# kxhit/vMAP

Measured on NVIDIA H100. Metric: training-step rays/sec at n_obj x n_rays x n_samples, higher is better.
Workload: dtype fp16

## Files before the change

### vmap_b200/csrc/k_step_fused.cuh

```cuda
#pragma once
#include <string>
#include <cmath>
#include "common.cuh"
#include "k_step_fp32.cuh"
#include "umma_ptx.cuh"
#include "k_umma_image.cuh"

struct FusedExtra {
  float* partials;
  unsigned int* finish_sync;
  const int* counts_in;
  int* counts_pub;
  int fuse_adam;
  float* p; float* m; float* v;
  __half* image_out; const int* img_index; int img_halves;
  int* step_counter;
  float step_size, bc2_sqrt;
  double lr, b1d, b2d;
  float log_b1, log_b2;
  const float2* bc_table;
  int bc_n;
  float lr_wd, one_m_b1, b2, one_m_b2, eps;
  int guard_loss;
  int* status;
// ... 20 lines not shown
  int on[3];
  int fin, skip;
  float step_size, bc2_sqrt;
  float lsum[4][4];
};
static_assert(sizeof(Misc) <= MISC_BYTES, "Misc");

__device__ __forceinline__ uint32_t pack_relu_h2(float lo, float hi) {
  uint32_t r;
  asm("cvt.rn.relu.satfinite.f16x2.f32 %0, %1, %2;" : "=r"(r) : "f"(hi), "f"(lo));
  return r;
}

__device__ __forceinline__ int wg_base(const VmbLayout& L, int blk, int lane, int& ld) {
  ld = 1;
  switch (blk) {
    case 0: {
      if (lane >= 96) return -1;
      const int j = um::emb1_col_to_j(lane);
      if (j == -2) return L.o_bin;
      if (j < 0) return -1;
      ld = VMB_E1; return L.o_Win + j;
    }
    case 1:
      if (lane < 32) { ld = 32; return L.o_Wm1 + lane; }
      return lane == 64 ? L.o_bm1 : -1;
    case 2: {
      if (lane < 32) { ld = 32 + VMB_E1; return L.o_Wcat + lane; }
      const int j = um::emb1_col_to_j(lane - 32);
      if (j == -2) return L.o_bcat;
      if (j < 0) return -1;
      ld = 32 + VMB_E1; return L.o_Wcat + 32 + j;
    }
    case 3:
      if (lane < 32) { ld = 32; return L.o_Wm2 + lane; }
      return lane == 64 + 42 ? L.o_bm2 : -1;
    default: {
      if (lane < 32) { ld = 32 + L.e2; return L.o_Wcl + lane; }
      if (lane >= 80) return -1;
      const int j2 = um::emb2_col_to_j2(lane - 32);
      if (j2 == -2) return L.o_bcl;
      if (j2 < 0) return -1;
      ld = 32 + L.e2; return L.o_Wcl + 32 + j2;
    }
  }
}

struct Mma {
  uint32_t a16, w16;
  int mh;

  static __device__ __forceinline__ uint64_t mk(uint32_t base16, uint32_t off, uint32_t lbo, uint32_t sbo) {
    const uint32_t lo = ((base16 + (off >> 4)) & 0x3FFFu) | ((lbo >> 4) << 16);
    return ((uint64_t)(sbo >> 4) << 32) | lo;
  }
  __device__ __forceinline__ uint64_t a_k(int fg, int ks) const { return mk(a16, fg * FGB + mh * 1024 + ks * 4096, 2048, 128); }
  __device__ __forceinline__ uint64_t xa_mn(int fg, int ks) const { return mk(a16, (fg + 8 * mh) * FGB + ks * 256, 128, 2048); }
  __device__ __forceinline__ uint64_t xb_mn(int fg, int ks) const { return mk(a16, fg * FGB + ks * 256, 128, 2048); }
  __device__ __forceinline__ uint64_t w_k(int off, int ks) const { return mk(w16, off + ks * 1024, 512, 128); }
  __device__ __forceinline__ uint64_t w16_k(int off, int ks) const { return mk(w16, off + ks * 512, 256, 128); }
  __device__ __forceinline__ uint64_t w_mn(int off, int ks) const { return mk(w16, off + ks * 256, 128, 512); }
  __device__ __forceinline__ uint64_t w16_mn(int off) const { return mk(w16, off, 128, 256); }

  __device__ __forceinline__ void wgrad32(float (&d)[16], int fgX, int fgDY) const {
#pragma unroll
    for (int ks = 0; ks < 8; ++ks) ptx::wgmma_n32<1, 1>(d, xa_mn(fgX, ks), xb_mn(fgDY, ks), 1u);
  }
  __device__ __forceinline__ void wgrad16(float (&d)[8], int fgX, int fgDY) const {
#pragma unroll
    for (int ks = 0; ks < 8; ++ks) ptx::wgmma_n16<1, 1>(d, xa_mn(fgX, ks), xb_mn(fgDY, ks), 1u);
  }
};

constexpr int MAX_CTAS = 192;
struct Ranges { int begin[MAX_CTAS + 1]; };
__device__ __forceinline__ int cta_of_pair(const Ranges& rg, int G, int pair) {
  int lo = 0, hi = G - 1;
  while (lo < hi) { const int mid = (lo + hi + 1) >> 1; if (rg.begin[mid] <= pair) lo = mid; else hi = mid - 1; }
  return lo;
}

}

template <int SC>
__global__ void __launch_bounds__(uf::NT, 1)
k_step_fused(StepParams a, FusedExtra x, VmbLayout L, const unsigned char* image, const __grid_constant__ uf::Ranges rg, int tpo, int npo, int nr, int rpw) {
  using namespace uf;
  extern __shared__ __align__(1024) unsigned char smem[];
  Misc* misc = reinterpret_cast<Misc*>(smem + SM_MISC);
  int* cnt = reinterpret_cast<int*>(smem + SM_CNT);
  const int tid = threadIdx.x, warp = tid >> 5, lane = tid & 31;
  const int S = SC ? SC : a.S, R = a.R;

  if (tid == 0) {
    ptx::mbar_init(&misc->wbar, 1);
    misc->on[0] = misc->on[1] = misc->on[2] = 1;
    ptx::mbar_init_fence();
  }
  const int G = gridDim.x;
  const long long gt_begin = rg.begin[blockIdx.x], gt_end = rg.begin[blockIdx.x + 1];
  __syncthreads();
  if (tid == 0 && gt_begin < gt_end) {
    ptx::mbar_arrive_expect_tx(&misc->wbar, um::IMG_BYTES);
    ptx::bulk_g2s(smem + SM_W, image + (size_t)(gt_begin / npo) * um::IMG_BYTES, um::IMG_BYTES, &misc->wbar);
  }
  const bool pub_counts = !x.counts_in && !a.fwd_only;
  unsigned int* gbar = x.finish_sync;
  if (pub_counts) {
    for (int b = blockIdx.x; b < a.B; b += G) {
      if (tid < 3) cnt[tid] = 0;
      __syncthreads();
      const unsigned char* s = a.sem + (size_t)b * a.sem_stride;
      const unsigned char* m = a.mask + (size_t)b * a.mask_stride;
      const bool vec = (((size_t)s | (size_t)m) & 3) == 0;
      const int nw = vec ? (R >> 2) : 0;
      auto nzb = [](uint32_t v) { v |= v >> 4; v |= v >> 2; v |= v >> 1; return v & 0x01010101u; };
      int nd = 0, no = 0, ns = 0;
      for (int w = tid; w < nw; w += NT) {
        const uint32_t sv = __ldg(reinterpret_cast<const uint32_t*>(s) + w), mv = __ldg(reinterpret_cast<const uint32_t*>(m) + w);
        const uint32_t o = nzb(sv);
        no += __popc(o); nd += __popc(o & nzb(mv)); ns += __popc(nzb(sv ^ 0x02020202u));
      }
      for (int r = (nw << 2) + tid; r < R; r += NT) {
        const int sv = s[r], mo = sv != 0;
        nd += (m[r] != 0) & mo; no += mo; ns += sv != 2;
      }
#pragma unroll
      for (int o = 16; o > 0; o >>= 1) {
        nd += __shfl_xor_sync(0xffffffffu, nd, o); no += __shfl_xor_sync(0xffffffffu, no, o); ns += __shfl_xor_sync(0xffffffffu, ns, o);
      }
      if (lane == 0) { atomicAdd(&cnt[0], nd); atomicAdd(&cnt[1], no); atomicAdd(&cnt[2], ns); }
      __syncthreads();
      if (tid == 0) {
        for (int k = 0; k < 3; ++k) {
          x.counts_pub[b * 4 + k] = cnt[k];
          if (cnt[k] == 0) atomicOr(&gbar[3 + k], 1u);
        }
        __threadfence();
        atomicAdd(&gbar[2], 1u);
      }
      __syncthreads();
    }
  } else if (!a.fwd_only) {
    for (int i = tid; i < a.B * 3; i += NT) {
      const int c = x.counts_in[(i / 3) * 4 + (i % 3)];
      cnt[i] = c;
      if (c == 0) misc->on[i % 3] = 0;
    }
  }
  __syncthreads();

  uint32_t wpar = 0;

  const int p = tid & 127, hsel = tid >> 7;
  const int quad = (warp & 3);
  const int rw = lane / S, sidx = lane - rw * S;
  const bool lane_used = rw < rpw;
  const int ray_in_tile = quad * rpw + rw;
  const int seg_lo = lane - sidx;
  unsigned char* act = smem + SM_ACT0;
  unsigned char* eg = smem + SM_EG;
  float* hd = reinterpret_cast<float*>(smem + SM_HD);
  const float* wf = reinterpret_cast<const float*>(smem + SM_W + um::IMG_F32);
  const float* Bd = wf + um::F_DIRS;
  const int cq = lane & 3, fr0 = 64 * hsel + 16 * quad + (lane >> 2);
  Mma mm;
  mm.a16 = ptx::smem_u32(act) >> 4;
  mm.w16 = ptx::smem_u32(smem + SM_W) >> 4;
  mm.mh = hsel;
  float wIN[16] = {}, wM1[16] = {}, wCAT[16] = {}, wM2[16] = {}, wCL[16] = {}, wHD[8] = {}, wDB[8] = {};
  const float on_d = misc->on[0] ? 1.f : 0.f, on_c = misc->on[1] ? 1.f : 0.f, on_o = misc->on[2] ? 1.f : 0.f;
  float w_d = 0.f, w_c = 0.f, w_o = 0.f;
  bool cnt_ready = !pub_counts;

  auto finish_rows = [&](int b, int i_lo, int i_hi, bool owner) -> int {
    const int c_first = cta_of_pair(rg, G, b * npo), c_last = cta_of_pair(rg, G, (b + 1) * npo - 1);
    const int nseg = c_last - c_first + 1;
    const float* P0 = x.partials + (size_t)(c_first + b) * L.stride;
    const size_t row = (size_t)b * L.stride;
    const int n4 = L.stride >> 2;
    const bool upd = a.backward != 0;
    if (warp == 0) {
      float s = 0.f;
      if (nseg <= 10) {
        const int k = lane / 3, j = lane - 3 * k;
        const float v = (k < nseg) ? __ldcg(P0 + (size_t)k * L.stride + L.P + j) : 0.f;
        for (int kk = 0; kk < nseg; ++kk) s += __shfl_sync(0xffffffffu, v, kk * 3 + (lane < 3 ? lane : 0));
      } else if (lane < 3) {
        for (int k = 0; k < nseg; ++k) s += __ldcg(P0 + (size_t)k * L.stride + L.P + lane);
      }
      const float l_d = __shfl_sync(0xffffffffu, s, 0), l_c = __shfl_sync(0xffffffffu, s, 1), l_o = __shfl_sync(0xffffffffu, s, 2);
      if (lane == 0) {
        const float tot = l_d + a.cs * l_c + a.os * l_o;
        if (owner) { float* lt = a.loss_terms + b * 4; lt[0] = l_d; lt[1] = l_c; lt[2] = l_o; lt[3] = tot; }
        int bad = 0;
        if (x.guard_loss) {
          if (l_d > 100000.f || l_c > 100000.f || l_o > 100000.f) bad |= 1;
          if (!(tot == tot) || fabsf(tot) > 3.0e38f) bad |= 2;
          if (bad && x.status && owner) atomicOr(x.status, bad);
        }
        misc->skip = bad;
        if (x.fuse_adam && x.step_counter) {
          const int t = x.step_counter[b] + 1;
          if (t < x.bc_n) {
            const float2 bc = x.bc_table[t];
            misc->step_size = (float)x.lr / bc.x;
            misc->bc2_sqrt = bc.y;
          } else {
            misc->step_size = (float)x.lr / (-expm1f((float)t * x.log_b1));
            misc->bc2_sqrt = sqrtf(-expm1f((float)t * x.log_b2));
          }
        } else {
          misc->step_size = x.step_size; misc->bc2_sqrt = x.bc2_sqrt;
        }
      }
    }
    __syncthreads();
    const int sk = misc->skip;
    if (upd && !(sk && x.fuse_adam)) {
      const float step_size = misc->step_size, bc2_sqrt = misc->bc2_sqrt;
      for (int c4 = i_lo + tid; c4 < i_hi; c4 += NT) {
        const float4* src = reinterpret_cast<const float4*>(P0) + c4;
        float4 pp, mm = make_float4(0.f, 0.f, 0.f, 0.f), vv = mm;
        if (x.fuse_adam) {
          pp = *(reinterpret_cast<const float4*>(x.p + row) + c4);
          mm = *(reinterpret_cast<const float4*>(x.m + row) + c4);
          vv = *(reinterpret_cast<const float4*>(x.v + row) + c4);
        } else {
          pp = *(reinterpret_cast<const float4*>(a.grads + row) + c4);
        }
        float4 gsum = make_float4(0.f, 0.f, 0.f, 0.f);
#pragma unroll 1
        for (int k0 = 0; k0 < nseg; k0 += 4) {
          float4 u[4];
#pragma unroll
// ... 43 lines not shown
    gt += p1 - p0;
    const int t0 = 2 * p0, t1 = min(2 * p1, tpo);

    um::mbar_wait_or_trap(&misc->wbar, wpar);
    wpar ^= 1;

    float ls_d = 0.f, ls_c = 0.f, ls_o = 0.f;
    {
    const float isc = 1.0f / a.scale[b];
    bool seg_w = false;
    if (x.counts_in && !a.fwd_only) {
      w_d = on_d / ((float)cnt[b * 3 + 0] + 1e-10f);
      w_c = on_c / ((float)cnt[b * 3 + 1] + 1e-10f);
      w_o = on_o / ((float)cnt[b * 3 + 2] + 1e-10f);
    }

#define OPERANDS_READY() do { ptx::fence_async_smem(); __syncthreads(); ptx::wgmma_fence(); } while (0)
#define MMA_DONE() do { ptx::wgmma_commit(); ptx::wgmma_wait<0>(); } while (0)
    auto epi_relu = [&](const float (&v)[16], int bias_off, int fg) {
#pragma unroll
      for (int j = 0; j < 4; ++j) {
        const float2 bb = *reinterpret_cast<const float2*>(wf + bias_off + 8 * j + 2 * cq);
        unsigned char* dst = act + (fg + j) * FGB + fr0 * 16 + cq * 4;
        *reinterpret_cast<uint32_t*>(dst) = pack_relu_h2(v[4 * j] + bb.x, v[4 * j + 1] + bb.y);
        *reinterpret_cast<uint32_t*>(dst + 128) = pack_relu_h2(v[4 * j + 2] + bb.x, v[4 * j + 3] + bb.y);
      }
    };
    auto epi_dgrad = [&](const float (&v)[16], int fg_h, int fg_out) {
#pragma unroll
      for (int j = 0; j < 4; ++j) {
        const int off = j * FGB + fr0 * 16 + cq * 4;
        const uint32_t h0 = *reinterpret_cast<const uint32_t*>(act + fg_h * FGB + off);
        const uint32_t h1 = *reinterpret_cast<const uint32_t*>(act + fg_h * FGB + off + 128);
        *reinterpret_cast<uint32_t*>(act + fg_out * FGB + off) = um::gate_h2(um::pack_h2(v[4 * j], v[4 * j + 1]), h0);
        *reinterpret_cast<uint32_t*>(act + fg_out * FGB + off + 128) = um::gate_h2(um::pack_h2(v[4 * j + 2], v[4 * j + 3]), h1);
      }
    };
    auto eg_store = [&](const auto& v, int blk0) {
      constexpr int NJ = (int)(sizeof(v) / 16);
#pragma unroll
      for (int j = 0; j < NJ; ++j) {
        float* d = reinterpret_cast<float*>(eg + (blk0 + 2 * j + (cq >> 1)) * FGB + fr0 * 16 + (cq & 1) * 8);
        *reinterpret_cast<float2*>(d) = make_float2(v[4 * j], v[4 * j + 1]);
        *reinterpret_cast<float2*>(d + 32) = make_float2(v[4 * j + 2], v[4 * j + 3]);
      }
    };
    auto eg_load8 = [&](int blk, float (&o)[8]) {
      const float4 u0 = *reinterpret_cast<const float4*>(eg + blk * FGB + p * 16);
      const float4 u1 = *reinterpret_cast<const float4*>(eg + (blk + 1) * FGB + p * 16);
      o[0] = u0.x; o[1] = u0.y; o[2] = u0.z; o[3] = u0.w; o[4] = u1.x; o[5] = u1.y; o[6] = u1.z; o[7] = u1.w;
    };

    float nx = 0.f, ny = 0.f, nz = 0.f, nzv = 0.f, n_gd = 0.f, n_c0 = 0.f, n_c1 = 0.f, n_c2 = 0.f;
    int n_sem = 0, n_msk = 0;
    bool n_live = false;
    const float* pcs_b = a.pcs + (size_t)b * a.pcs_stride + (size_t)sidx * 3;
    const float* z_b = a.z + (size_t)b * a.z_stride + sidx;
    const float* gd_b = a.gt_depth + (size_t)b * a.gt_depth_stride;
    const float* gc_b = a.gt_colour + (size_t)b * a.gt_colour_stride;
    const unsigned char* sem_b = a.sem + (size_t)b * a.sem_stride;
    const unsigned char* msk_b = a.mask + (size_t)b * a.mask_stride;
    const bool want_targets = hsel == 0 && !a.fwd_only;
    auto prefetch = [&](int t) {
      nx = ny = nz = nzv = 0.f; n_gd = n_c0 = n_c1 = n_c2 = 0.f; n_sem = 0; n_msk = 0; n_live = false;
      if (t >= t1 || !lane_used) return;
      const int ray = t * nr + ray_in_tile;
      if (ray >= R) return;
      const size_t pi = (size_t)ray * S;
      const float* pp = pcs_b + pi * 3;
      nx = pp[0]; ny = pp[1]; nz = pp[2];
      if (want_targets) {
        nzv = z_b[pi];
        n_gd = gd_b[ray];
        const float* gcp = gc_b + (size_t)ray * 3;
        n_c0 = gcp[0]; n_c1 = gcp[1]; n_c2 = gcp[2];
        n_sem = sem_b[ray];
        n_msk = msk_b[ray];
      }
      n_live = true;
    };
    prefetch(t0);

    for (int t = t0; t < t1; ++t) {
      const int ray = t * nr + ray_in_tile;
      const float t0x = nx * isc, t1x = ny * isc, t2x = nz * isc, zv = nzv;
      const uint64_t tp0 = um::pk2(t0x, t0x), tp1 = um::pk2(t1x, t1x), tp2 = um::pk2(t2x, t2x);
      const float gd = n_gd, gc0 = n_c0, gc1 = n_c1, gc2 = n_c2;
      const int sv = n_sem, mv = n_msk;
      const bool live = n_live;
      prefetch(t + 1);
      {
        uint4* e1 = reinterpret_cast<uint4*>(act + FG_E1 * FGB + p * 16);
        uint4* e2 = reinterpret_cast<uint4*>(act + FG_E2 * FGB + p * 16);
        const int q0 = hsel ? 3 : 0, q1 = hsel ? 5 : 3;
        uint64_t s01, s23, c01, c23;
        {
          uint64_t pj01, pj23;
          um::project4(Bd, q0, tp0, tp1, tp2, pj01, pj23);
          um::sincos4_x2(pj01, pj23, s01, s23, c01, c23);
        }
#pragma unroll 1
        for (int q = q0; q < q1; ++q) {
          float sv[4][6];
          uint64_t ns01 = 0, ns23 = 0, nc01 = 0, nc23 = 0;
          if (q + 1 < q1) {
            uint64_t pj01, pj23;
            um::project4(Bd, q + 1, tp0, tp1, tp2, pj01, pj23);
            um::sincos4_x2(pj01, pj23, ns01, ns23, nc01, nc23);
          }
          um::sin_doubling4_x2(s01, s23, c01, c23, sv);
          s01 = ns01; s23 = ns23; c01 = nc01; c23 = nc23;
          const uint4 ua = make_uint4(um::pack_h2(sv[0][0], sv[0][1]), um::pack_h2(sv[0][2], sv[0][3]), um::pack_h2(sv[1][0], sv[1][1]), um::pack_h2(sv[1][2], sv[1][3]));
          const uint4 ub = make_uint4(um::pack_h2(sv[2][0], sv[2][1]), um::pack_h2(sv[2][2], sv[2][3]), um::pack_h2(sv[3][0], sv[3][1]), um::pack_h2(sv[3][2], sv[3][3]));
          const uint4 uc = make_uint4(um::pack_h2(sv[0][4], sv[0][5]), um::pack_h2(sv[1][4], sv[1][5]), um::pack_h2(sv[2][4], sv[2][5]), um::pack_h2(sv[3][4], sv[3][5]));
          e1[(2 * q + 1) * 128] = ua; e1[(2 * q + 2) * 128] = ub; e2[q * 128] = uc;
        }
        if (hsel) {
          float s[6];
          um::sin_ladder(fmaf(Bd[2 * um::DIRS_PITCH + 20], t2x, fmaf(Bd[um::DIRS_PITCH + 20], t1x, Bd[20] * t0x)), s);
          const uint4 u0 = make_uint4(um::pack_h2(1.0f, t0x), um::pack_h2(t1x, t2x), um::pack_h2(s[0], s[1]), um::pack_h2(s[2], s[3]));
          const uint4 u5 = make_uint4(um::pack_h2(s[4], s[5]), um::pack_h2(1.0f, 0.f), 0u, 0u);
          e1[0] = u0;
          e2[5 * 128] = u5;
          e1[11 * 128] = make_uint4(0u, 0u, 0u, 0u);
          uint4* dh = reinterpret_cast<uint4*>(act + FG_DH * FGB + p * 16);
          dh[0] = make_uint4(0u, 0u, 0u, 0u); dh[128] = make_uint4(0u, 0u, 0u, 0u);
        }
      }
      float acc[16], hacc[8];
      OPERANDS_READY();
#pragma unroll
      for (int ks = 0; ks < 6; ++ks) ptx::wgmma_n32<0, 0>(acc, mm.a_k(FG_E1, ks), mm.w_k(um::IMG_WIN, ks), ks > 0);
      MMA_DONE();
      epi_relu(acc, um::F_BIN, FG_FC1);
      OPERANDS_READY();
#pragma unroll
      for (int ks = 0; ks < 2; ++ks) ptx::wgmma_n32<0, 0>(acc, mm.a_k(FG_FC1, ks), mm.w_k(um::IMG_WM1, ks), ks > 0);
      MMA_DONE();
      epi_relu(acc, um::F_BM1, FG_FC2);
      OPERANDS_READY();
#pragma unroll
      for (int ks = 0; ks < 8; ++ks) ptx::wgmma_n32<0, 0>(acc, mm.a_k(FG_FC2, ks), mm.w_k(um::IMG_WCAT, ks), ks > 0);
      MMA_DONE();
      epi_relu(acc, um::F_BCAT, FG_FC3);
      OPERANDS_READY();
#pragma unroll
      for (int ks = 0; ks < 2; ++ks) ptx::wgmma_n32<0, 0>(acc, mm.a_k(FG_FC3, ks), mm.w_k(um::IMG_WM2, ks), ks > 0);
      MMA_DONE();
      epi_relu(acc, um::F_BM2, FG_FC4);
      OPERANDS_READY();
#pragma unroll
      for (int ks = 0; ks < 5; ++ks) ptx::wgmma_n32<0, 0>(acc, mm.a_k(FG_FC4, ks), mm.w_k(um::IMG_WCL, ks), ks > 0);
#pragma unroll
      for (int ks = 0; ks < 2; ++ks) ptx::wgmma_n16<0, 0>(hacc, mm.a_k(FG_FC4, ks), mm.w16_k(um::IMG_WA16, ks), ks > 0);
      MMA_DONE();
      epi_relu(acc, um::F_BCL, FG_HC);
      if (cq == 0) { hd[fr0 * 4] = hacc[0]; hd[(fr0 + 8) * 4] = hacc[2]; }
      OPERANDS_READY();
#pragma unroll
      for (int ks = 0; ks < 2; ++ks) ptx::wgmma_n16<0, 0>(hacc, mm.a_k(FG_HC, ks), mm.w16_k(um::IMG_WOC16, ks), ks > 0);
      MMA_DONE();
      if (cq == 0) { hd[fr0 * 4 + 1] = hacc[1]; hd[(fr0 + 8) * 4 + 1] = hacc[3]; }
      if (cq == 1) { hd[fr0 * 4 + 2] = hacc[0]; hd[fr0 * 4 + 3] = hacc[1]; hd[(fr0 + 8) * 4 + 2] = hacc[2]; hd[(fr0 + 8) * 4 + 3] = hacc[3]; }
      __syncthreads();
      auto raysum = [&](float v) {
#pragma unroll
        for (int off = 1; off < 32; off <<= 1) {
          if (off < S) { const float u = __shfl_down_sync(0xffffffffu, v, off); if (sidx + off < S) v += u; }
        }
        return __shfl_sync(0xffffffffu, v, seg_lo);
      };
      float araw = 0.f, occ = 0.f, fr = 1.f, Tr = 1.f, w = 0.f, D = 0.f, O = 0.f, V = 0.f;
      if (hsel == 0) {
        if (pub_counts && !seg_w) {
          if (!cnt_ready) {
            const volatile unsigned int* pubd = gbar + 2;
            unsigned int spins = 0;
            while (*pubd < (unsigned int)a.B) { if (++spins > 2000000000u) __trap(); }
            __threadfence();
            cnt_ready = true;
          }
          const volatile unsigned int* ef = gbar + 3;
          const volatile int* cp = x.counts_pub + b * 4;
          w_d = (ef[0] ? 0.f : 1.f) / ((float)cp[0] + 1e-10f);
          w_c = (ef[1] ? 0.f : 1.f) / ((float)cp[1] + 1e-10f);
          w_o = (ef[2] ? 0.f : 1.f) / ((float)cp[2] + 1e-10f);
          seg_w = true;
        }
        araw = (hd[p * 4] + wf[um::F_BA]) * 10.0f;
        occ = um::fast_sigmoid(araw);
        if (!a.fwd_only) {
          if (!live) occ = 0.f;
          fr = 1.f - occ + 1e-10f;
          float inc = fr;
#pragma unroll
          for (int off = 1; off < 32; off <<= 1) {
            if (off < S) { const float u = __shfl_up_sync(0xffffffffu, inc, off); if (sidx >= off) inc *= u; }
          }
          Tr = __shfl_up_sync(0xffffffffu, inc, 1);
          if (sidx == 0) Tr = 1.f;
          w = occ * Tr;
          D = raysum(w * zv); O = raysum(w);
          const float dz = zv - D;
          V = raysum(w * dz * dz);
        }
      }
      if (hsel == 0) {
        const float4 hv = *reinterpret_cast<const float4*>(hd + p * 4);
        const float c0 = um::fast_sigmoid(hv.y + wf[um::F_BOC + 0]), c1 = um::fast_sigmoid(hv.z + wf[um::F_BOC + 1]),
                    c2 = um::fast_sigmoid(hv.w + wf[um::F_BOC + 2]);
        if (a.fwd_only) {
          if (live) {
            const size_t n = (size_t)ray * S + sidx;
            a.out_alpha[(size_t)b * a.alpha_stride + n] = araw;
            float* oc = a.out_colour + (size_t)b * a.colour_stride + n * 3;
            oc[0] = c0; oc[1] = c1; oc[2] = c2;
          }
        } else {
          const float C0 = raysum(w * c0), C1 = raysum(w * c1), C2 = raysum(w * c2);
          const float m_o = (live && sv != 0) ? 1.f : 0.f, m_s = (live && sv != 2) ? 1.f : 0.f, m_d = (mv != 0) ? m_o : 0.f;
          const float info = 1.f / (sqrtf(V) + 1e-4f);
          const float e_d = D - gd, e_o = O - m_o, e_c0 = C0 - gc0, e_c1 = C1 - gc1, e_c2 = C2 - gc2;
          if (live && sidx == 0) {
            if (a.r_depth) a.r_depth[(size_t)b * R + ray] = D;
            if (a.r_var) a.r_var[(size_t)b * R + ray] = V;
            if (a.r_opacity) a.r_opacity[(size_t)b * R + ray] = O;
            if (a.r_colour) { float* rc = a.r_colour + ((size_t)b * R + ray) * 3; rc[0] = C0; rc[1] = C1; rc[2] = C2; }
            ls_d += w_d * fabsf(e_d) * m_d * info;
            ls_c += w_c * (fabsf(e_c0) + fabsf(e_c1) + fabsf(e_c2)) * m_o;
            ls_o += w_o * fabsf(e_o) * m_s;
          }
          if (a.backward) {
            const float gD = LS * w_d * vmb_sign(e_d) * m_d * info;
            const float kc = LS * w_c * a.cs * m_o;
            const float gC0 = kc * vmb_sign(e_c0), gC1 = kc * vmb_sign(e_c1), gC2 = kc * vmb_sign(e_c2);
            const float gO = LS * w_o * a.os * vmb_sign(e_o) * m_s;
            const float Gs = fmaf(gD, zv, fmaf(gC0, c0, fmaf(gC1, c1, fmaf(gC2, c2, gO))));
            float suf = Gs * w;
#pragma unroll
            for (int off = 1; off < 32; off <<= 1) {
              if (off < S) { const float u = __shfl_down_sync(0xffffffffu, suf, off); if (sidx + off < S) suf += u; }
            }
            float sx = __shfl_down_sync(0xffffffffu, suf, 1);
            if (sidx + 1 >= S) sx = 0.f;
            const float docc = Gs * Tr - __fdividef(sx, fr);
            const float da = 10.0f * docc * occ * (1.f - occ);
            if (live)
              *reinterpret_cast<uint2*>(act + FG_DH * FGB + p * 16) =
                  make_uint2(um::pack_h2(da, gC0 * w * c0 * (1.f - c0)), um::pack_h2(gC1 * w * c1 * (1.f - c1), gC2 * w * c2 * (1.f - c2)));
          }
        }
      }
      if (a.fwd_only || !a.backward) { __syncthreads(); continue; }
      OPERANDS_READY();
      ptx::wgmma_n32<0, 1>(acc, mm.a_k(FG_DH, 0), mm.w16_mn(um::IMG_WOC16), 0u);
      mm.wgrad16(wHD, FG_FC4, FG_DH);
      MMA_DONE();
      epi_dgrad(acc, FG_HC, FG_Z);
      OPERANDS_READY();
#pragma unroll
      for (int ks = 0; ks < 2; ++ks) ptx::wgmma_n32<0, 1>(acc, mm.a_k(FG_Z, ks), mm.w_mn(um::IMG_WCL, ks), ks > 0);
      ptx::wgmma_n32<0, 1>(acc, mm.a_k(FG_DH, 0), mm.w16_mn(um::IMG_WA16), 1u);
      mm.wgrad32(wCL, FG_FC4, FG_Z);
      MMA_DONE();
      epi_dgrad(acc, FG_FC4, FG_HC);
      OPERANDS_READY();
#pragma unroll
      for (int ks = 0; ks < 2; ++ks) ptx::wgmma_n32<0, 1>(acc, mm.a_k(FG_HC, ks), mm.w_mn(um::IMG_WM2, ks), ks > 0);
      mm.wgrad32(wM2, FG_FC3, FG_HC);
      MMA_DONE();
      epi_dgrad(acc, FG_FC3, FG_FC4);
      OPERANDS_READY();
#pragma unroll
      for (int ks = 0; ks < 2; ++ks) ptx::wgmma_n32<0, 1>(acc, mm.a_k(FG_FC4, ks), mm.w_mn(um::IMG_WCAT, ks), ks > 0);
      mm.wgrad32(wCAT, FG_FC2, FG_FC4);
      MMA_DONE();
      epi_dgrad(acc, FG_FC2, FG_HC);
      OPERANDS_READY();
#pragma unroll
      for (int ks = 0; ks < 2; ++ks) ptx::wgmma_n32<0, 1>(acc, mm.a_k(FG_HC, ks), mm.w_mn(um::IMG_WM1, ks), ks > 0);
      mm.wgrad32(wM1, FG_FC1, FG_HC);
      MMA_DONE();
      epi_dgrad(acc, FG_FC1, FG_FC3);
      OPERANDS_READY();
#pragma unroll
      for (int c = 0; c < 3; ++c) {
#pragma unroll
        for (int ks = 0; ks < 2; ++ks) ptx::wgmma_n32<0, 1>(acc, mm.a_k(FG_FC4, ks), mm.w_mn(um::IMG_WCAT + (4 + 4 * c) * 512, ks), ks > 0);
#pragma unroll
        for (int ks = 0; ks < 2; ++ks) ptx::wgmma_n32<0, 1>(acc, mm.a_k(FG_FC3, ks), mm.w_mn(um::IMG_WIN + 4 * c * 512, ks), 1u);
        MMA_DONE();
        eg_store(acc, 8 * c);
        ptx::wgmma_fence();
      }
#pragma unroll
      for (int ks = 0; ks < 2; ++ks) ptx::wgmma_n32<0, 1>(acc, mm.a_k(FG_Z, ks), mm.w_mn(um::IMG_WCL + 4 * 512, ks), ks > 0);
#pragma unroll
      for (int ks = 0; ks < 2; ++ks) ptx::wgmma_n16<0, 1>(hacc, mm.a_k(FG_Z, ks), mm.w_mn(um::IMG_WCL + 8 * 512, ks), ks > 0);
      mm.wgrad32(wIN, FG_E1, FG_FC3);
      MMA_DONE();
      eg_store(acc, EG_E2);
      eg_store(hacc, EG_E2 + 8);
      __syncthreads();
      {
        const int q0 = hsel ? 3 : 0, q1 = hsel ? 5 : 3;
        uint64_t c01, c23;
        {
          uint64_t pj01, pj23;
          um::project4(Bd, q0, tp0, tp1, tp2, pj01, pj23);
          um::cos4_x2(pj01, pj23, c01, c23);
        }
#pragma unroll 1
        for (int q = q0; q < q1; ++q) {
          float g1a[8], g1b[8], g2[8];
          eg_load8(4 * q + 2, g1a);
          eg_load8(4 * q + 4, g1b);
          eg_load8(EG_E2 + 2 * q, g2);
          float cv[4][6], dp[4];
          uint64_t nc01 = 0, nc23 = 0;
          if (q + 1 < q1) {
            uint64_t pj01, pj23;
            um::project4(Bd, q + 1, tp0, tp1, tp2, pj01, pj23);
            um::cos4_x2(pj01, pj23, nc01, nc23);
          }
          um::cos_doubling4_x2(c01, c23, cv);
          c01 = nc01; c23 = nc23;
#pragma unroll
          for (int dd = 0; dd < 4; ++dd) {
            const float* g1 = (dd < 2) ? (g1a + dd * 4) : (g1b + (dd - 2) * 4);
            float d = g1[0] * cv[dd][0];
            d = fmaf(2.f * g1[1], cv[dd][1], d);
            d = fmaf(4.f * g1[2], cv[dd][2], d);
            d = fmaf(8.f * g1[3], cv[dd][3], d);
            d = fmaf(16.f * g2[dd * 2], cv[dd][4], d);
            d = fmaf(32.f * g2[dd * 2 + 1], cv[dd][5], d);
            dp[dd] = d * VMB_PI_F;
          }
          *reinterpret_cast<uint2*>(act + (FG_DPR + (q >> 1)) * FGB + p * 16 + (q & 1) * 8) =
              make_uint2(um::pack_h2(dp[0], dp[1]), um::pack_h2(dp[2], dp[3]));
        }
        if (hsel) {
          float g1[8], g2[8], c[6];
          eg_load8(0, g1);
          eg_load8(EG_E2 + 10, g2);
          um::cos_ladder(fmaf(Bd[2 * um::DIRS_PITCH + 20], t2x, fmaf(Bd[um::DIRS_PITCH + 20], t1x, Bd[20] * t0x)), c);
          float d = g1[4] * c[0];
          d = fmaf(2.f * g1[5], c[1], d); d = fmaf(4.f * g1[6], c[2], d); d = fmaf(8.f * g1[7], c[3], d);
          d = fmaf(16.f * g2[0], c[4], d); d = fmaf(32.f * g2[1], c[5], d);
          *reinterpret_cast<uint2*>(act + (FG_DPR + 2) * FGB + p * 16 + 8) = make_uint2(um::pack_h2(d * VMB_PI_F, 0.f), 0u);
        }
      }
      OPERANDS_READY();
      mm.wgrad16(wDB, FG_DPR, FG_E1);
      MMA_DONE();
      __syncthreads();
    }
#undef OPERANDS_READY
#undef MMA_DONE
    }
    if (a.fwd_only) {
      __syncthreads();
      if (tid == 0 && gt < gt_end) {
        ptx::mbar_arrive_expect_tx(&misc->wbar, um::IMG_BYTES);
        ptx::bulk_g2s(smem + SM_W, image + (size_t)(gt / npo) * um::IMG_BYTES, um::IMG_BYTES, &misc->wbar);
      }
      continue;
    }
    ls_d = warp_sum(ls_d); ls_c = warp_sum(ls_c); ls_o = warp_sum(ls_o);
    if (hsel == 0 && lane == 0) { float* l = misc->lsum[quad]; l[0] = ls_d; l[1] = ls_c; l[2] = ls_o; }
    __syncthreads();
    if (tid == 0 && gt < gt_end) {
      ptx::mbar_arrive_expect_tx(&misc->wbar, um::IMG_BYTES);
      ptx::bulk_g2s(smem + SM_W, image + (size_t)(gt / npo) * um::IMG_BYTES, um::IMG_BYTES, &misc->wbar);
    }
    float* Pr = reinterpret_cast<float*>(smem + SM_ACT0);
    if (tid < 3) {
      float s = 0.f;
#pragma unroll
      for (int w8 = 0; w8 < 4; ++w8) s += misc->lsum[w8][tid];
      Pr[L.P + tid] = s;
    }
    if (a.backward) {
      auto put = [&](float (&d)[16], int blk) {
#pragma unroll
        for (int i = 0; i < 2; ++i) {
          int ld;
          const int base = wg_base(L, blk, fr0 + 8 * i, ld);
          if (base >= 0) {
#pragma unroll
            for (int j = 0; j < 4; ++j)
#pragma unroll
              for (int e = 0; e < 2; ++e) Pr[base + (8 * j + 2 * cq + e) * ld] = d[4 * j + 2 * i + e] * INV_LS;
          }
        }
#pragma unroll
        for (int k = 0; k < 16; ++k) d[k] = 0.f;
      };
      put(wIN, 0); put(wM1, 1); put(wCAT, 2); put(wM2, 3); put(wCL, 4);
#pragma unroll
      for (int i = 0; i < 2; ++i) {
        const int ln = fr0 + 8 * i;
#pragma unroll
        for (int e = 0; e < 2; ++e) {
          const int col = 2 * cq + e;
          const float vh = wHD[2 * i + e] * INV_LS, vb = wDB[2 * i + e] * INV_LS;
          if (col == 0) {
            if (ln < 32) Pr[L.o_Wa + ln] = vh;
            else if (ln == 32 + 42) Pr[L.o_ba] = vh;
          } else if (col < 4) {
            if (ln == 32 + 42) Pr[L.o_boc + col - 1] = vh;
            else if (ln >= 80 && ln < 112) Pr[L.o_Woc + (col - 1) * 32 + (ln - 80)] = vh;
            if (ln < VMB_NDIRS) Pr[L.o_B + ln * 3 + col - 1] = vb;
          }
        }
      }
#pragma unroll
      for (int k = 0; k < 8; ++k) { wHD[k] = 0.f; wDB[k] = 0.f; }
    }
    __syncthreads();
    {
      float4* dst = reinterpret_cast<float4*>(x.partials + (size_t)(blockIdx.x + b) * L.stride);
      const float4* src = reinterpret_cast<const float4*>(Pr);
      for (int i = tid; i < (L.stride >> 2); i += NT) dst[i] = src[i];
    }
    __syncthreads();
  }

  if (!a.fwd_only) {
    __threadfence();
    __syncthreads();
    if (tid == 0) {
      atomicAdd(&gbar[0], 1u);
      unsigned int spins = 0;
      while (atomicAdd(&gbar[0], 0u) < (unsigned int)G) { __nanosleep(32); if (++spins > 400000000u) __trap(); }
    }
    __syncthreads();
    __threadfence();
    const int n4 = L.stride >> 2;
    const long long W = (long long)a.B * n4;
    const long long lo = (W * blockIdx.x) / G, hi = (W * (blockIdx.x + 1)) / G;
    for (int b = (int)(lo / n4); (long long)b * n4 < hi; ++b) {
      const int i_lo = (int)(max(lo, (long long)b * n4) - (long long)b * n4);
      const int i_hi = (int)(min(hi, (long long)(b + 1) * n4) - (long long)b * n4);
      const int skip = finish_rows(b, i_lo, i_hi, i_lo == 0);
      if (i_lo == 0 && tid == 0) gbar[6 + b] = (unsigned int)skip;
    }
    __threadfence();
    __syncthreads();
    if (tid == 0) misc->fin = (atomicAdd(&gbar[1], 1u) + 1u == (unsigned int)G) ? 1 : 0;
    __syncthreads();
    if (misc->fin) {
      __threadfence();
      if (x.fuse_adam && x.step_counter && a.backward)
        for (int b = tid; b < a.B; b += NT) if (gbar[6 + b] == 0u) x.step_counter[b] += 1;
      if (x.loss_sum && warp == 0) {
        float s = 0.f;
        for (int b = lane; b < a.B; b += 32) s += __ldcg(a.loss_terms + b * 4 + 3);
        s = warp_sum(s);
        if (lane == 0) *x.loss_sum = s;
      }
      __syncthreads();
      if (tid == 0) { gbar[0] = 0u; gbar[1] = 0u; gbar[2] = 0u; gbar[3] = 0u; gbar[4] = 0u; gbar[5] = 0u; }
    }
  }

}

static int fused_rows_needed(int n_obj, int n_sm) { return n_obj + n_sm; }

static void fused_partition(int B, int npo, int G, uf::Ranges& rg) {
  const long long T = (long long)B * npo;
  double beta = 0.0;
  if (T >= 2LL * G) {
    const long long rounds = (T + G - 1) / G;
    for (double cand : {1.0, 0.7, 0.4}) {
      if ((long long)std::ceil(((double)T + cand * (B - 1)) / G - 1e-9) <= rounds) { beta = cand; break; }
    }
  }
  const double V = (double)T + beta * (B - 1);
  int c = 0;
  rg.begin[0] = 0;
  for (long long p = 0; p < T; ++p) {
    const double x = (double)p + beta * (double)(p / npo);
    while (c < G - 1 && x >= V * (c + 1) / G && p > rg.begin[c] && T - p >= G - 1 - c) rg.begin[++c] = (int)p;
    if (T - p - 1 == G - 1 - c && c < G - 1) {
      for (long long q = p + 1; q < T; ++q) rg.begin[++c] = (int)q;
      break;
    }
  }
  while (c < G) rg.begin[++c] = (int)T;
}

static int fused_launch_step(const VmbLayout& L, const StepParams& sp, const FusedExtra& fx, const void* image, int n_sm,
                             cudaStream_t st, std::string& err) {
  using namespace uf;
  if (L.H != 32 || L.nfreq != 6) { err = "fused step kernel: hidden must be 32 and n_freq 6"; return -4; }
  if (sp.S < 1 || sp.S > 32) { err = "fused step kernel: n_samples must be in [1, 32]"; return -4; }
  if (!sp.fwd_only && sp.B > MAX_OBJ_SMEM) { err = "fused step kernel: too many objects for the in-kernel mask counts"; return -4; }
  static bool attr_set[64] = {};
  int dev = 0;
  cudaGetDevice(&dev);
  const int smem_bytes = SM_CNT + (sp.fwd_only ? 0 : sp.B * 12) + 16;
  if (!attr_set[dev & 63]) {
    cudaError_t e = cudaFuncSetAttribute(k_step_fused<0>, cudaFuncAttributeMaxDynamicSharedMemorySize, SMEM_MAX);
    if (e == cudaSuccess) e = cudaFuncSetAttribute(k_step_fused<10>, cudaFuncAttributeMaxDynamicSharedMemorySize, SMEM_MAX);
    if (e == cudaSuccess) e = cudaFuncSetAttribute(k_step_fused<14>, cudaFuncAttributeMaxDynamicSharedMemorySize, SMEM_MAX);
    if (e != cudaSuccess) { err = std::string("cudaFuncSetAttribute(k_step_fused): ") + cudaGetErrorString(e); return -2; }
    attr_set[dev & 63] = true;
  }
  const int rpw = 32 / sp.S;
  const int nr = 4 * rpw;
  const int tpo = (sp.R + nr - 1) / nr;
  const int npo = (tpo + 1) / 2;
  const long long T = (long long)npo * sp.B;
  if (T > 0x7fffffffLL) { err = "fused step kernel: too many tiles"; return -1; }
  long long grid = T;
  if (grid > n_sm) grid = n_sm;
  if (grid > MAX_CTAS) grid = MAX_CTAS;
  if (grid < 1) grid = 1;
  Ranges rg;
  fused_partition(sp.B, npo, (int)grid, rg);
  const unsigned char* img = (const unsigned char*)image;
  cudaLaunchConfig_t cfg;
  memset(&cfg, 0, sizeof(cfg));
  cfg.gridDim = dim3((unsigned)grid); cfg.blockDim = dim3(NT); cfg.dynamicSmemBytes = smem_bytes; cfg.stream = st;
  cudaLaunchAttribute attr[1];
  attr[0].id = cudaLaunchAttributeCooperative;
  attr[0].val.cooperative = sp.fwd_only ? 0 : 1;
  cfg.attrs = attr; cfg.numAttrs = 1;
  cudaError_t e;
  if (sp.S == 10)      e = cudaLaunchKernelEx(&cfg, k_step_fused<10>, sp, fx, L, img, rg, tpo, npo, nr, rpw);
  else if (sp.S == 14) e = cudaLaunchKernelEx(&cfg, k_step_fused<14>, sp, fx, L, img, rg, tpo, npo, nr, rpw);
  else                 e = cudaLaunchKernelEx(&cfg, k_step_fused<0>, sp, fx, L, img, rg, tpo, npo, nr, rpw);
  if (e == cudaSuccess) e = cudaGetLastError();
  if (e != cudaSuccess) { err = std::string("k_step_fused launch: ") + cudaGetErrorString(e); return -2; }
  return 0;
}
```

### vmap_b200/csrc/vmb_api.cu

```cuda
#include <cstdio>
#include <cstdlib>
#include <cstring>
#include <cmath>
#include <string>
#include <type_traits>
#include <vector>

#include "../../include/vmap_b200.h"
#include "common.cuh"
#include "k_step_fp32.cuh"
#include "k_adam.cuh"
#include "k_sampler.cuh"
#include "k_ingest.cuh"
#include "k_umma_image.cuh"
#include "k_step_fused.cuh"
#include "k_gemm_umma.cuh"
#include "k_layerwise.cuh"
#include "k_mesh.cuh"
#include "k_eval.cuh"
#include "k_assoc.cuh"
#include "k_hull.cuh"
#include "k_render.cuh"
#include "k_track.cuh"
#include "k_ba.cuh"
#include "k_track_lw.cuh"

struct vmb_handle {
  int device, max_obj, H, nfreq;
  int n_sm;
  VmbLayout L;
  int* d_counts;
  int* d_img_index;
  unsigned int* d_ticket;
  unsigned int* d_smax;
  float* d_partials;
  unsigned int* d_finish_sync;
  float2* d_bc;
  double bc_b1, bc_b2;
  int img_halves;
  bool umma_ok;
  bool lw_ok;
  lw::Workspace ws;
  lw::Workspace ws_fwd;
  mesh::Workspace ws_mesh;
  eval3d::Workspace ws_eval;
  assoc::Workspace ws_assoc;
  hull::Workspace ws_hull;
  render::Workspace ws_render;
  lw::TrackWorkspace ws_track;
  lw::TrackWorkspace ws_ba;
  std::string err;
};

static thread_local std::string g_err;

static int fail(vmb_handle* h, int code, const std::string& msg) {
  if (h) h->err = msg;
  g_err = msg;
  return code;
}
#define CUDA_TRY(h, expr)                                                                  \
  do {                                                                                     \
    cudaError_t e_ = (expr);                                                               \
    if (e_ != cudaSuccess)                                                                 \
      return fail(h, VMB_E_CUDA, std::string(#expr) + ": " + cudaGetErrorString(e_));      \
  } while (0)

template <int H, int TP>
static int launch_fp32(vmb_handle* h, const StepParams& sp, long long n_tiles_x, cudaStream_t st) {
  const size_t smem = step_fp32_smem<H, TP>(h->L);
  static bool attr_set[64] = {};
  if (!attr_set[h->device & 63]) {
    CUDA_TRY(h, cudaFuncSetAttribute(k_step_fp32<H, TP>, cudaFuncAttributeMaxDynamicSharedMemorySize, (int)smem));
    attr_set[h->device & 63] = true;
  }
  dim3 grid((unsigned)n_tiles_x, (unsigned)sp.B);
  k_step_fp32<H, TP><<<grid, 128, smem, st>>>(sp, h->L);
  CUDA_TRY(h, cudaGetLastError());
  return VMB_OK;
}

static int dispatch_fp32(vmb_handle* h, const StepParams& sp, cudaStream_t st) {
  const int TP = (h->H == 32) ? 128 : (h->H == 256 ? 32 : 64);
  if (sp.S > TP) return fail(h, VMB_E_UNSUPPORTED, "fp32 step kernel: n_samples exceeds the tile size for this hidden size");
  const int nr = TP / sp.S;
  const long long tiles = ((long long)sp.R + nr - 1) / nr;
  if (tiles > 0x7fffffffLL || sp.B > 65535) return fail(h, VMB_E_ARG, "grid too large");
  switch (h->H) {
    case 32:  return launch_fp32<32, 128>(h, sp, tiles, st);
    case 64:  return launch_fp32<64, 64>(h, sp, tiles, st);
    case 128: return launch_fp32<128, 64>(h, sp, tiles, st);
    case 256: return launch_fp32<256, 32>(h, sp, tiles, st);
  }
  return fail(h, VMB_E_UNSUPPORTED, "unsupported hidden size");
}

extern "C" {

const char* vmb_version(void) { return "vmap_b200 0.1 (sm_90a)"; }

int vmb_param_count(int hidden, int n_freq) {
  if (hidden <= 0 || n_freq < 4 || n_freq > VMB_MAX_FREQ) return VMB_E_ARG;
  return vmb_make_layout(hidden, n_freq).P;
}
int vmb_param_stride(int hidden, int n_freq) {
  if (hidden <= 0 || n_freq < 4 || n_freq > VMB_MAX_FREQ) return VMB_E_ARG;
  return vmb_make_layout(hidden, n_freq).stride;
}
int vmb_param_offsets(int hidden, int n_freq, int* offsets, int* sizes) {
  if (hidden <= 0 || n_freq < 4 || n_freq > VMB_MAX_FREQ || !offsets || !sizes) return VMB_E_ARG;
  const VmbLayout L = vmb_make_layout(hidden, n_freq);
  const int H = hidden;
  const int off[VMB_N_TENSORS] = {L.o_Win, L.o_bin, L.o_Wm1, L.o_bm1, L.o_Wcat, L.o_bcat, L.o_Wm2, L.o_bm2,
                                  L.o_Wa, L.o_ba, L.o_Wcl, L.o_bcl, L.o_Woc, L.o_boc, L.o_B};
  const int sz[VMB_N_TENSORS] = {H * VMB_E1, H, H * H, H, H * (H + VMB_E1), H, H * H, H,
                                 H, 1, H * (H + L.e2), H, 3 * H, 3, VMB_NDIRS * 3};
  for (int i = 0; i < VMB_N_TENSORS; ++i) { offsets[i] = off[i]; sizes[i] = sz[i]; }
  return VMB_OK;
}
int vmb_image_bytes(int hidden, int n_freq) {
  if (hidden == 32 && n_freq == 6) return umma_image_bytes();
  if ((hidden == 64 || hidden == 128 || hidden == 256) && n_freq == 6) return (int)(2 * lw::img_halves(hidden));
  return 0;
}

const char* vmb_last_error(const vmb_handle* h) { return h ? h->err.c_str() : g_err.c_str(); }

int vmb_create(vmb_handle** out, int device, int max_obj, int hidden, int n_freq) {
  if (!out || max_obj <= 0) return fail(nullptr, VMB_E_ARG, "vmb_create: bad arguments");
  if (!(hidden == 32 || hidden == 64 || hidden == 128 || hidden == 256))
    return fail(nullptr, VMB_E_UNSUPPORTED, "vmb_create: hidden must be 32, 64, 128 or 256");
  if (n_freq < 4 || n_freq > VMB_MAX_FREQ) return fail(nullptr, VMB_E_ARG, "vmb_create: n_freq must be in [4,8]");
  CUDA_TRY(nullptr, cudaSetDevice(device));
  vmb_handle* h = new vmb_handle();
  h->device = device; h->max_obj = max_obj; h->H = hidden; h->nfreq = n_freq;
  h->n_sm = 132;
  cudaDeviceGetAttribute(&h->n_sm, cudaDevAttrMultiProcessorCount, device);
  h->L = vmb_make_layout(hidden, n_freq);
  h->d_counts = nullptr; h->d_img_index = nullptr; h->d_ticket = nullptr; h->d_smax = nullptr; h->d_partials = nullptr; h->d_finish_sync = nullptr; h->d_bc = nullptr; h->bc_b1 = h->bc_b2 = -1.0; h->img_halves = 0; h->umma_ok = false; h->lw_ok = false;
  cudaError_t e = cudaMalloc(&h->d_counts, sizeof(int) * 4 * max_obj);
  if (e == cudaSuccess) e = cudaMalloc(&h->d_ticket, sizeof(unsigned int));
  if (e == cudaSuccess) e = cudaMemset(h->d_ticket, 0, sizeof(unsigned int));
  if (e == cudaSuccess) e = cudaMalloc(&h->d_smax, sizeof(unsigned int) * (size_t)max_obj);
  if (e != cudaSuccess) { delete h; return fail(nullptr, VMB_E_NOMEM, cudaGetErrorString(e)); }
  if (hidden == 32 && n_freq == 6) {
    std::vector<int> idx(h->L.P);
    umma_fill_image_index(h->L, idx.data());
    h->img_halves = umma_image_bytes() / 2;
    e = cudaMalloc(&h->d_img_index, sizeof(int) * h->L.P);
    if (e == cudaSuccess) e = cudaMemcpy(h->d_img_index, idx.data(), sizeof(int) * h->L.P, cudaMemcpyHostToDevice);
    if (e != cudaSuccess) { cudaFree(h->d_counts); delete h; return fail(nullptr, VMB_E_CUDA, cudaGetErrorString(e)); }
    h->umma_ok = true;
  } else if ((hidden == 64 || hidden == 128 || hidden == 256) && n_freq == 6) {
    std::vector<int> idx(h->L.P);
    lw::fill_image_index(h->L, idx.data());
    h->img_halves = (int)lw::img_halves(hidden);
    e = cudaMalloc(&h->d_img_index, sizeof(int) * h->L.P);
    if (e == cudaSuccess) e = cudaMemcpy(h->d_img_index, idx.data(), sizeof(int) * h->L.P, cudaMemcpyHostToDevice);
    if (e != cudaSuccess) { cudaFree(h->d_counts); delete h; return fail(nullptr, VMB_E_CUDA, cudaGetErrorString(e)); }
    h->lw_ok = true;
  }
  *out = h;
  return VMB_OK;
}

void vmb_destroy(vmb_handle* h) {
  if (!h) return;
  cudaSetDevice(h->device);
  if (h->d_counts) cudaFree(h->d_counts);
  if (h->d_img_index) cudaFree(h->d_img_index);
  if (h->d_ticket) cudaFree(h->d_ticket);
  if (h->d_smax) cudaFree(h->d_smax);
  if (h->d_partials) cudaFree(h->d_partials);
  if (h->d_finish_sync) cudaFree(h->d_finish_sync);
  if (h->d_bc) cudaFree(h->d_bc);
  h->ws.release(); h->ws.destroy_streams();
  h->ws_fwd.release(); h->ws_fwd.destroy_streams();
  h->ws_mesh.release();
  h->ws_eval.release();
  h->ws_assoc.release();
  h->ws_hull.release();
  h->ws_render.release();
// ... 1186 lines not shown
```

Measured before the change: 148.6 million.

## Overlap backward dgrad epilogues with wgrad MMAs and batch ray reductions

In the backward pass, the data-gradient wgmma and the weight-gradient wgmma are now committed as separate groups. The dgrad epilogue runs after waiting only for the first group, so it overlaps the wgrad MMAs still in flight. In the forward pass, the color sigmoids are computed earlier and the five per-ray segment sums are batched into one interleaved shuffle reduction instead of separate ones. Compile-time-disabled clock64 tracing hooks and a trace readback API are also added. This raises register pressure and depends on the commit/wait grouping preserving correct smem hazards.

```diff
diff --git a/vmap_b200/csrc/k_step_fused.cuh b/vmap_b200/csrc/k_step_fused.cuh
--- a/vmap_b200/csrc/k_step_fused.cuh
+++ b/vmap_b200/csrc/k_step_fused.cuh
@@ -126,6 +126,20 @@
 
 }
 
+#if VMB_FUSED_TRACE
+namespace uf {
+constexpr int TR_TILES = 32, TR_EV = 64;
+__device__ long long g_trace[MAX_CTAS][2][TR_TILES + 1][TR_EV];
+}
+#define TR_AT(slot, ev) do { if (lane == 0 && (warp & 3) == 0 && (slot) <= TR_TILES) \
+                               uf::g_trace[blockIdx.x][warp >> 2][slot][ev] = clock64(); } while (0)
+#define TR(ev) TR_AT(tr_slot < TR_TILES ? tr_slot : TR_TILES + 1, ev)
+#define TRL(ev) TR_AT(TR_TILES, ev)
+#else
+#define TR(ev) do {} while (0)
+#define TRL(ev) do {} while (0)
+#endif
+
 template <int SC>
 __global__ void __launch_bounds__(uf::NT, 1)
 k_step_fused(StepParams a, FusedExtra x, VmbLayout L, const unsigned char* image, const __grid_constant__ uf::Ranges rg, int tpo, int npo, int nr, int rpw) {
@@ -135,6 +149,7 @@
   int* cnt = reinterpret_cast<int*>(smem + SM_CNT);
   const int tid = threadIdx.x, warp = tid >> 5, lane = tid & 31;
   const int S = SC ? SC : a.S, R = a.R;
+  TRL(0);
 
   if (tid == 0) {
     ptx::mbar_init(&misc->wbar, 1);
@@ -193,8 +208,12 @@
     }
   }
   __syncthreads();
+  TRL(1);
 
   uint32_t wpar = 0;
+#if VMB_FUSED_TRACE
+  int tr_n = 0, tr_seg = 0;
+#endif
 
   const int p = tid & 127, hsel = tid >> 7;
   const int quad = (warp & 3);
@@ -404,6 +423,10 @@
     prefetch(t0);
 
     for (int t = t0; t < t1; ++t) {
+#if VMB_FUSED_TRACE
+      const int tr_slot = tr_n++;
+#endif
+      TR(0);
       const int ray = t * nr + ray_in_tile;
       const float t0x = nx * isc, t1x = ny * isc, t2x = nz * isc, zv = nzv;
       const uint64_t tp0 = um::pk2(t0x, t0x), tp1 = um::pk2(t1x, t1x), tp2 = um::pk2(t2x, t2x);
@@ -449,42 +472,62 @@
           dh[0] = make_uint4(0u, 0u, 0u, 0u); dh[128] = make_uint4(0u, 0u, 0u, 0u);
         }
       }
+      TR(1);
       float acc[16], hacc[8];
       OPERANDS_READY();
+      TR(2);
 #pragma unroll
       for (int ks = 0; ks < 6; ++ks) ptx::wgmma_n32<0, 0>(acc, mm.a_k(FG_E1, ks), mm.w_k(um::IMG_WIN, ks), ks > 0);
       MMA_DONE();
+      TR(3);
       epi_relu(acc, um::F_BIN, FG_FC1);
-      OPERANDS_READY();
+      TR(4);
+      OPERANDS_READY();
+      TR(5);
 #pragma unroll
       for (int ks = 0; ks < 2; ++ks) ptx::wgmma_n32<0, 0>(acc, mm.a_k(FG_FC1, ks), mm.w_k(um::IMG_WM1, ks), ks > 0);
       MMA_DONE();
+      TR(6);
       epi_relu(acc, um::F_BM1, FG_FC2);
-      OPERANDS_READY();
+      TR(7);
+      OPERANDS_READY();
+      TR(8);
 #pragma unroll
       for (int ks = 0; ks < 8; ++ks) ptx::wgmma_n32<0, 0>(acc, mm.a_k(FG_FC2, ks), mm.w_k(um::IMG_WCAT, ks), ks > 0);
       MMA_DONE();
+      TR(9);
       epi_relu(acc, um::F_BCAT, FG_FC3);
-      OPERANDS_READY();
+      TR(10);
+      OPERANDS_READY();
+      TR(11);
 #pragma unroll
       for (int ks = 0; ks < 2; ++ks) ptx::wgmma_n32<0, 0>(acc, mm.a_k(FG_FC3, ks), mm.w_k(um::IMG_WM2, ks), ks > 0);
       MMA_DONE();
+      TR(12);
       epi_relu(acc, um::F_BM2, FG_FC4);
-      OPERANDS_READY();
+      TR(13);
+      OPERANDS_READY();
+      TR(14);
 #pragma unroll
       for (int ks = 0; ks < 5; ++ks) ptx::wgmma_n32<0, 0>(acc, mm.a_k(FG_FC4, ks), mm.w_k(um::IMG_WCL, ks), ks > 0);
 #pragma unroll
       for (int ks = 0; ks < 2; ++ks) ptx::wgmma_n16<0, 0>(hacc, mm.a_k(FG_FC4, ks), mm.w16_k(um::IMG_WA16, ks), ks > 0);
       MMA_DONE();
+      TR(15);
       epi_relu(acc, um::F_BCL, FG_HC);
       if (cq == 0) { hd[fr0 * 4] = hacc[0]; hd[(fr0 + 8) * 4] = hacc[2]; }
-      OPERANDS_READY();
+      TR(16);
+      OPERANDS_READY();
+      TR(17);
 #pragma unroll
       for (int ks = 0; ks < 2; ++ks) ptx::wgmma_n16<0, 0>(hacc, mm.a_k(FG_HC, ks), mm.w16_k(um::IMG_WOC16, ks), ks > 0);
       MMA_DONE();
+      TR(18);
       if (cq == 0) { hd[fr0 * 4 + 1] = hacc[1]; hd[(fr0 + 8) * 4 + 1] = hacc[3]; }
       if (cq == 1) { hd[fr0 * 4 + 2] = hacc[0]; hd[fr0 * 4 + 3] = hacc[1]; hd[(fr0 + 8) * 4 + 2] = hacc[2]; hd[(fr0 + 8) * 4 + 3] = hacc[3]; }
+      TR(19);
       __syncthreads();
+      TR(20);
       auto raysum = [&](float v) {
 #pragma unroll
         for (int off = 1; off < 32; off <<= 1) {
@@ -492,7 +535,23 @@
         }
         return __shfl_sync(0xffffffffu, v, seg_lo);
       };
+      auto raysum_n = [&](auto& v) {
+        constexpr int N = (int)(sizeof(v) / sizeof(float));
+#pragma unroll
+        for (int off = 1; off < 32; off <<= 1) {
+          if (off < S) {
+            float u[N];
+#pragma unroll
+            for (int i = 0; i < N; ++i) u[i] = __shfl_down_sync(0xffffffffu, v[i], off);
+#pragma unroll
+            for (int i = 0; i < N; ++i) if (sidx + off < S) v[i] += u[i];
+          }
+        }
+#pragma unroll
+        for (int i = 0; i < N; ++i) v[i] = __shfl_sync(0xffffffffu, v[i], seg_lo);
+      };
       float araw = 0.f, occ = 0.f, fr = 1.f, Tr = 1.f, w = 0.f, D = 0.f, O = 0.f, V = 0.f;
+      float c0 = 0.f, c1 = 0.f, c2 = 0.f, C0 = 0.f, C1 = 0.f, C2 = 0.f;
       if (hsel == 0) {
         if (pub_counts && !seg_w) {
           if (!cnt_ready) {
@@ -509,8 +568,11 @@
           w_o = (ef[2] ? 0.f : 1.f) / ((float)cp[2] + 1e-10f);
           seg_w = true;
         }
-        araw = (hd[p * 4] + wf[um::F_BA]) * 10.0f;
+        const float4 hv = *reinterpret_cast<const float4*>(hd + p * 4);
+        araw = (hv.x + wf[um::F_BA]) * 10.0f;
         occ = um::fast_sigmoid(araw);
+        c0 = um::fast_sigmoid(hv.y + wf[um::F_BOC + 0]); c1 = um::fast_sigmoid(hv.z + wf[um::F_BOC + 1]);
+        c2 = um::fast_sigmoid(hv.w + wf[um::F_BOC + 2]);
         if (!a.fwd_only) {
           if (!live) occ = 0.f;
           fr = 1.f - occ + 1e-10f;
@@ -522,15 +584,14 @@
           Tr = __shfl_up_sync(0xffffffffu, inc, 1);
           if (sidx == 0) Tr = 1.f;
           w = occ * Tr;
-          D = raysum(w * zv); O = raysum(w);
+          float rs[5] = {w * zv, w, w * c0, w * c1, w * c2};
+          raysum_n(rs);
+          D = rs[0]; O = rs[1]; C0 = rs[2]; C1 = rs[3]; C2 = rs[4];
           const float dz = zv - D;
           V = raysum(w * dz * dz);
         }
       }
       if (hsel == 0) {
-        const float4 hv = *reinterpret_cast<const float4*>(hd + p * 4);
-        const float c0 = um::fast_sigmoid(hv.y + wf[um::F_BOC + 0]), c1 = um::fast_sigmoid(hv.z + wf[um::F_BOC + 1]),
-                    c2 = um::fast_sigmoid(hv.w + wf[um::F_BOC + 2]);
         if (a.fwd_only) {
           if (live) {
             const size_t n = (size_t)ray * S + sidx;
@@ -539,7 +600,6 @@
             oc[0] = c0; oc[1] = c1; oc[2] = c2;
           }
         } else {
-          const float C0 = raysum(w * c0), C1 = raysum(w * c1), C2 = raysum(w * c2);
           const float m_o = (live && sv != 0) ? 1.f : 0.f, m_s = (live && sv != 2) ? 1.f : 0.f, m_d = (mv != 0) ? m_o : 0.f;
           const float info = 1.f / (sqrtf(V) + 1e-4f);
           const float e_d = D - gd, e_o = O - m_o, e_c0 = C0 - gc0, e_c1 = C1 - gc1, e_c2 = C2 - gc2;
@@ -573,38 +633,70 @@
           }
         }
       }
+      TR(21);
       if (a.fwd_only || !a.backward) { __syncthreads(); continue; }
       OPERANDS_READY();
+      TR(22);
       ptx::wgmma_n32<0, 1>(acc, mm.a_k(FG_DH, 0), mm.w16_mn(um::IMG_WOC16), 0u);
+      ptx::wgmma_commit();
       mm.wgrad16(wHD, FG_FC4, FG_DH);
-      MMA_DONE();
+      ptx::wgmma_commit();
+      ptx::wgmma_wait<1>();
+      TR(23);
       epi_dgrad(acc, FG_HC, FG_Z);
-      OPERANDS_READY();
+      ptx::wgmma_wait<0>();
+      TR(24);
+      OPERANDS_READY();
+      TR(25);
 #pragma unroll
       for (int ks = 0; ks < 2; ++ks) ptx::wgmma_n32<0, 1>(acc, mm.a_k(FG_Z, ks), mm.w_mn(um::IMG_WCL, ks), ks > 0);
       ptx::wgmma_n32<0, 1>(acc, mm.a_k(FG_DH, 0), mm.w16_mn(um::IMG_WA16), 1u);
+      ptx::wgmma_commit();
       mm.wgrad32(wCL, FG_FC4, FG_Z);
-      MMA_DONE();
+      ptx::wgmma_commit();
+      ptx::wgmma_wait<1>();
+      TR(26);
       epi_dgrad(acc, FG_FC4, FG_HC);
-      OPERANDS_READY();
+      ptx::wgmma_wait<0>();
+      TR(27);
+      OPERANDS_READY();
+      TR(28);
 #pragma unroll
       for (int ks = 0; ks < 2; ++ks) ptx::wgmma_n32<0, 1>(acc, mm.a_k(FG_HC, ks), mm.w_mn(um::IMG_WM2, ks), ks > 0);
+      ptx::wgmma_commit();
       mm.wgrad32(wM2, FG_FC3, FG_HC);
-      MMA_DONE();
+      ptx::wgmma_commit();
+      ptx::wgmma_wait<1>();
+      TR(29);
       epi_dgrad(acc, FG_FC3, FG_FC4);
-      OPERANDS_READY();
+      ptx::wgmma_wait<0>();
+      TR(30);
+      OPERANDS_READY();
+      TR(31);
 #pragma unroll
       for (int ks = 0; ks < 2; ++ks) ptx::wgmma_n32<0, 1>(acc, mm.a_k(FG_FC4, ks), mm.w_mn(um::IMG_WCAT, ks), ks > 0);
+      ptx::wgmma_commit();
       mm.wgrad32(wCAT, FG_FC2, FG_FC4);
-      MMA_DONE();
+      ptx::wgmma_commit();
+      ptx::wgmma_wait<1>();
+      TR(32);
       epi_dgrad(acc, FG_FC2, FG_HC);
-      OPERANDS_READY();
+      ptx::wgmma_wait<0>();
+      TR(33);
+      OPERANDS_READY();
+      TR(34);
 #pragma unroll
       for (int ks = 0; ks < 2; ++ks) ptx::wgmma_n32<0, 1>(acc, mm.a_k(FG_HC, ks), mm.w_mn(um::IMG_WM1, ks), ks > 0);
+      ptx::wgmma_commit();
       mm.wgrad32(wM1, FG_FC1, FG_HC);
-      MMA_DONE();
+      ptx::wgmma_commit();
+      ptx::wgmma_wait<1>();
+      TR(35);
       epi_dgrad(acc, FG_FC1, FG_FC3);
-      OPERANDS_READY();
+      ptx::wgmma_wait<0>();
+      TR(36);
+      OPERANDS_READY();
+      TR(37);
 #pragma unroll
       for (int c = 0; c < 3; ++c) {
 #pragma unroll
@@ -612,6 +704,7 @@
 #pragma unroll
         for (int ks = 0; ks < 2; ++ks) ptx::wgmma_n32<0, 1>(acc, mm.a_k(FG_FC3, ks), mm.w_mn(um::IMG_WIN + 4 * c * 512, ks), 1u);
         MMA_DONE();
+        TR(38 + c);
         eg_store(acc, 8 * c);
         ptx::wgmma_fence();
       }
@@ -619,11 +712,17 @@
       for (int ks = 0; ks < 2; ++ks) ptx::wgmma_n32<0, 1>(acc, mm.a_k(FG_Z, ks), mm.w_mn(um::IMG_WCL + 4 * 512, ks), ks > 0);
 #pragma unroll
       for (int ks = 0; ks < 2; ++ks) ptx::wgmma_n16<0, 1>(hacc, mm.a_k(FG_Z, ks), mm.w_mn(um::IMG_WCL + 8 * 512, ks), ks > 0);
+      ptx::wgmma_commit();
       mm.wgrad32(wIN, FG_E1, FG_FC3);
-      MMA_DONE();
+      ptx::wgmma_commit();
+      ptx::wgmma_wait<1>();
+      TR(41);
       eg_store(acc, EG_E2);
       eg_store(hacc, EG_E2 + 8);
+      ptx::wgmma_wait<0>();
+      TR(42);
       __syncthreads();
+      TR(43);
       {
         const int q0 = hsel ? 3 : 0, q1 = hsel ? 5 : 3;
         uint64_t c01, c23;
@@ -672,10 +771,14 @@
           *reinterpret_cast<uint2*>(act + (FG_DPR + 2) * FGB + p * 16 + 8) = make_uint2(um::pack_h2(d * VMB_PI_F, 0.f), 0u);
         }
       }
-      OPERANDS_READY();
+      TR(44);
+      OPERANDS_READY();
+      TR(45);
       mm.wgrad16(wDB, FG_DPR, FG_E1);
       MMA_DONE();
+      TR(46);
       __syncthreads();
+      TR(47);
     }
 #undef OPERANDS_READY
 #undef MMA_DONE
@@ -688,6 +791,10 @@
       }
       continue;
     }
+#if VMB_FUSED_TRACE
+    const int tr_k = tr_seg < 8 ? tr_seg++ : 8;
+#endif
+    TRL(2 + 2 * tr_k);
     ls_d = warp_sum(ls_d); ls_c = warp_sum(ls_c); ls_o = warp_sum(ls_o);
     if (hsel == 0 && lane == 0) { float* l = misc->lsum[quad]; l[0] = ls_d; l[1] = ls_c; l[2] = ls_o; }
     __syncthreads();
@@ -746,17 +853,20 @@
       for (int i = tid; i < (L.stride >> 2); i += NT) dst[i] = src[i];
     }
     __syncthreads();
+    TRL(3 + 2 * tr_k);
   }
 
   if (!a.fwd_only) {
     __threadfence();
     __syncthreads();
+    TRL(20);
     if (tid == 0) {
       atomicAdd(&gbar[0], 1u);
       unsigned int spins = 0;
       while (atomicAdd(&gbar[0], 0u) < (unsigned int)G) { __nanosleep(32); if (++spins > 400000000u) __trap(); }
     }
     __syncthreads();
+    TRL(21);
     __threadfence();
     const int n4 = L.stride >> 2;
     const long long W = (long long)a.B * n4;
@@ -784,6 +894,7 @@
       __syncthreads();
       if (tid == 0) { gbar[0] = 0u; gbar[1] = 0u; gbar[2] = 0u; gbar[3] = 0u; gbar[4] = 0u; gbar[5] = 0u; }
     }
+    TRL(22);
   }
 
 }
diff --git a/vmap_b200/csrc/vmb_api.cu b/vmap_b200/csrc/vmb_api.cu
--- a/vmap_b200/csrc/vmb_api.cu
+++ b/vmap_b200/csrc/vmb_api.cu
@@ -98,6 +98,20 @@
 extern "C" {
 
 const char* vmb_version(void) { return "vmap_b200 0.1 (sm_90a)"; }
+
+#if VMB_FUSED_TRACE
+int vmb_fused_trace_read(void* dst, long long bytes) {
+  if (bytes != (long long)sizeof(uf::g_trace)) return VMB_E_ARG;
+  cudaError_t e = cudaMemcpyFromSymbol(dst, uf::g_trace, sizeof(uf::g_trace));
+  if (e == cudaSuccess) {
+    void* d = nullptr;
+    e = cudaGetSymbolAddress(&d, uf::g_trace);
+    if (e == cudaSuccess) e = cudaMemset(d, 0, sizeof(uf::g_trace));
+    if (e == cudaSuccess) e = cudaDeviceSynchronize();
+  }
+  return e == cudaSuccess ? VMB_OK : VMB_E_CUDA;
+}
+#endif
 
 int vmb_param_count(int hidden, int n_freq) {
   if (hidden <= 0 || n_freq < 4 || n_freq > VMB_MAX_FREQ) return VMB_E_ARG;
```

Result: no change. 149.5 million, median of 6 (+0.6%).
